# openai/Video-Pre-Training

Hardware: AMD Instinct MI355X
Metric: frames/sec (fwd) [+ bc_step.ms_per_step], 2x policy, 128x128x3 seq=128 (higher is better)
Workload: dtype bf16; 1 GPU; foundation-model-2x policy forward (IMPALA CNN + 4-layer banded transformer + heads), batch=64 seq=128 uint8 128x128x3 frames per GPU, KV memory carried, random-init weights; global_batch=64, seq_len=128, parallelism=dp1 replicas (no collective in forward; BC step: gradient all-reduce)

## Files before the change

### video-pre-training_amd/csrc/vpt_transformer.hip

```cpp
#include "vpt_common.h"
#include "vpt_kernels.h"

__global__ __launch_bounds__(256) void vpt_layernorm_kernel(VptLayerNormArgs a) {
  const int lane = threadIdx.x & 63;
  const int row = blockIdx.x * 4 + (threadIdx.x >> 6);
  if (row >= a.M) return;
  const float* x = a.x + (size_t)row * a.D;
  const int n4 = a.D >> 2;
  float s = 0.f;
  for (int i = lane; i < n4; i += 64) {
    f32x4 v = *(const f32x4*)(x + 4 * i);
    if (a.relu_in) { v.x = fmaxf(v.x, 0.f); v.y = fmaxf(v.y, 0.f); v.z = fmaxf(v.z, 0.f); v.w = fmaxf(v.w, 0.f); }
    s += (v.x + v.y) + (v.z + v.w);
  }
  const float mean = wave_sum(s) / (float)a.D;
  float ss = 0.f;
  for (int i = lane; i < n4; i += 64) {
    f32x4 v = *(const f32x4*)(x + 4 * i);
    if (a.relu_in) { v.x = fmaxf(v.x, 0.f); v.y = fmaxf(v.y, 0.f); v.z = fmaxf(v.z, 0.f); v.w = fmaxf(v.w, 0.f); }
    const float d0 = v.x - mean, d1 = v.y - mean, d2 = v.z - mean, d3 = v.w - mean;
    ss += (d0 * d0 + d1 * d1) + (d2 * d2 + d3 * d3);
  }
  const float rstd = rsqrtf(wave_sum(ss) / (float)a.D + VPT_NORM_EPS);
  for (int i = lane; i < n4; i += 64) {
    f32x4 v = *(const f32x4*)(x + 4 * i);
    if (a.relu_in) { v.x = fmaxf(v.x, 0.f); v.y = fmaxf(v.y, 0.f); v.z = fmaxf(v.z, 0.f); v.w = fmaxf(v.w, 0.f); }
    const f32x4 g = *(const f32x4*)(a.gain + 4 * i), b = *(const f32x4*)(a.bias + 4 * i);
    f32x4 y;
    y.x = fmaf((v.x - mean) * rstd, g.x, b.x);
    y.y = fmaf((v.y - mean) * rstd, g.y, b.y);
    y.z = fmaf((v.z - mean) * rstd, g.z, b.z);
    y.w = fmaf((v.w - mean) * rstd, g.w, b.w);
    if (a.out_f32) *(f32x4*)(a.out_f32 + (size_t)row * a.D + 4 * i) = y;
    if (a.out_bf16) {
      u32x2 p = {pack_op16x2(y.x, y.y), pack_op16x2(y.z, y.w)};
      *(u32x2*)(a.out_bf16 + (size_t)row * a.D + 4 * i) = p;
    }
  }
}

extern "C" int vpt_layernorm_launch(const VptLayerNormArgs* a, hipStream_t stream) {
  if (a->M <= 0 || (a->D & 3)) return -1;
  hipLaunchKernelGGL(vpt_layernorm_kernel, dim3((a->M + 3) >> 2), dim3(256), 0, stream, *a);
  return hipGetLastError() == hipSuccess ? 0 : -3;
}

#define ATT_DH 128
#define ATT_QT 32
#define ATT_NK 160
#define ATT_RS (ATT_DH + 4)
#define ATT_SS 164
#define ATT_S_OFF 0
#define ATT_R_OFF (ATT_S_OFF + ATT_QT * ATT_SS)
#define ATT_B_OFF (ATT_R_OFF + ATT_QT * 10)
#define ATT_SC_OFF (ATT_B_OFF + 10 * 129)
#define ATT_QL_OFF (ATT_SC_OFF + ATT_QT)
#define ATT_PT_OFF ((ATT_QL_OFF + ATT_QT + 3) & ~3)
#define ATT_FLOATS (ATT_PT_OFF + 4 * 16 * 64)

__global__ __launch_bounds__(256) void vpt_attn_kernel(VptAttnArgs a) {
  extern __shared__ __attribute__((aligned(16))) float sm[];
  float* Ss = sm + ATT_S_OFF;
  float* Rs = sm + ATT_R_OFF;
  float* Bs = sm + ATT_B_OFF;
  float* Sc = sm + ATT_SC_OFF;
  int* Ql = (int*)(sm + ATT_QL_OFF);

  const int tid = threadIdx.x, lane = tid & 63, w = __builtin_amdgcn_readfirstlane(tid >> 6);
  const int b = blockIdx.y / a.heads, h = blockIdx.y - b * a.heads;
  const int q0 = blockIdx.x * ATT_QT;
  const int maxlen = a.maxlen, t = a.t, hid = a.hid;
  const size_t tok0 = (size_t)b * t;
  const int jbase = a.causal ? q0 + 1 : 0;

  for (int idx = tid; idx < ATT_QT * 10; idx += 256) {
    const int r = idx / 10, n = idx - r * 10;
    Rs[idx] = (a.causal && q0 + r < t) ? a.qkvr[(tok0 + q0 + r) * a.ld + 3 * hid + h * 10 + n] : 0.f;
  }
  for (int idx = tid; idx < 10 * maxlen; idx += 256) Bs[idx] = a.b_nd[idx];
  if (tid < ATT_QT) Ql[tid] = (a.qlo && q0 + tid < t) ? a.qlo[tok0 + q0 + tid] : 0;
  __syncthreads();

  const int l31 = lane & 31, hi = lane >> 5;
  auto kv_row = [&](int j, int which) -> const float* {
    if (j < maxlen) return (which == 1 ? a.kmem : a.vmem) + ((size_t)b * maxlen + j) * hid + h * ATT_DH;
    if (j - maxlen < t) return a.qkvr + (tok0 + j - maxlen) * a.ld + which * hid + h * ATT_DH;
    return nullptr;
  };
  {
    f32x16 acc, acc4;
#pragma unroll
    for (int r = 0; r < 16; ++r) { acc[r] = 0.f; acc4[r] = 0.f; }
    const f32x4 z4 = {0.f, 0.f, 0.f, 0.f};
    const float* qa = (q0 + l31 < t) ? a.qkvr + (tok0 + q0 + l31) * a.ld + h * ATT_DH + 4 * hi : nullptr;
    const float* kr = kv_row(jbase + w * 32 + l31, 1);
    const float* kr4 = kv_row(jbase + 128 + l31, 1);
    const float* kb = kr ? kr + 4 * hi : nullptr;
    const float* kb4 = kr4 ? kr4 + 4 * hi : nullptr;
#pragma unroll 8
    for (int g = 0; g < 16; ++g) {
      const f32x4 q4 = qa ? *(const f32x4*)(qa + 8 * g) : z4, k4 = kb ? *(const f32x4*)(kb + 8 * g) : z4;
      acc = __builtin_amdgcn_mfma_f32_32x32x2f32(q4.x, k4.x, acc, 0, 0, 0);
      acc = __builtin_amdgcn_mfma_f32_32x32x2f32(q4.y, k4.y, acc, 0, 0, 0);
      acc = __builtin_amdgcn_mfma_f32_32x32x2f32(q4.z, k4.z, acc, 0, 0, 0);
      acc = __builtin_amdgcn_mfma_f32_32x32x2f32(q4.w, k4.w, acc, 0, 0, 0);
    }
#pragma unroll
    for (int g4 = 0; g4 < 4; ++g4) {
      const int g = 4 * w + g4;
      const f32x4 q4 = qa ? *(const f32x4*)(qa + 8 * g) : z4, k4 = kb4 ? *(const f32x4*)(kb4 + 8 * g) : z4;
      acc4 = __builtin_amdgcn_mfma_f32_32x32x2f32(q4.x, k4.x, acc4, 0, 0, 0);
      acc4 = __builtin_amdgcn_mfma_f32_32x32x2f32(q4.y, k4.y, acc4, 0, 0, 0);
      acc4 = __builtin_amdgcn_mfma_f32_32x32x2f32(q4.z, k4.z, acc4, 0, 0, 0);
      acc4 = __builtin_amdgcn_mfma_f32_32x32x2f32(q4.w, k4.w, acc4, 0, 0, 0);
    }
    float* Pt = sm + ATT_PT_OFF;
#pragma unroll
    for (int r = 0; r < 16; ++r) Pt[(w * 16 + r) * 64 + lane] = acc4[r];
    __syncthreads();
    auto finish = [&](int kk, int r, float dot) {
      const int qi = (r & 3) + 8 * (r >> 2) + 4 * hi;
      const bool qvalid = (q0 + qi) < t;
      const int off = maxlen - 1 + qi - kk;
      const int j = jbase + kk;
      bool vis = a.causal ? (qvalid && off >= 0 && off < maxlen) : (qvalid && kk < t);
      if (vis && a.causal && j < maxlen) vis = a.memvalid[(size_t)b * maxlen + j] != 0;
      vis = vis && j >= Ql[qi];
      float sc = -3.0e38f;
      if (vis) {
        float rb = 0.f;
        if (a.causal) {
#pragma unroll
          for (int n = 0; n < 10; ++n) rb = fmaf(Rs[qi * 10 + n], Bs[n * maxlen + off], rb);
        }
        sc = dot * (1.0f / ATT_DH) + rb;
      }
      Ss[qi * ATT_SS + kk] = sc;
    };
#pragma unroll
    for (int r = 0; r < 16; ++r) finish(w * 32 + l31, r, acc[r]);
#pragma unroll
    for (int r4 = 0; r4 < 4; ++r4) {
      const int r = 4 * w + r4;
      const float dot = (Pt[(0 * 16 + r) * 64 + lane] + Pt[(1 * 16 + r) * 64 + lane]) + (Pt[(2 * 16 + r) * 64 + lane] + Pt[(3 * 16 + r) * 64 + lane]);
      finish(128 + l31, r, dot);
    }
  }
  __syncthreads();
  for (int r = w * 8; r < w * 8 + 8; ++r) {
    float* srow = Ss + r * ATT_SS;
    const float s0 = srow[lane], s1 = srow[lane + 64], s2 = (lane + 128 < ATT_NK) ? srow[lane + 128] : -3.0e38f;
    const float m = wave_max(fmaxf(s0, fmaxf(s1, s2)));
    const float e0 = (s0 > -1.0e38f) ? expf(s0 - m) : 0.f;
    const float e1 = (s1 > -1.0e38f) ? expf(s1 - m) : 0.f;
    const float e2 = (s2 > -1.0e38f) ? expf(s2 - m) : 0.f;
    const float tot = wave_sum(e0 + e1 + e2);
    srow[lane] = e0;
    srow[lane + 64] = e1;
    if (lane + 128 < ATT_NK) srow[lane + 128] = e2;
    if (lane == 0) Sc[r] = (tot > 0.f) ? 1.0f / tot : 0.f;
  }
  __syncthreads();

  {
    f32x16 o;
#pragma unroll
    for (int r = 0; r < 16; ++r) o[r] = 0.f;
    const float* pa = Ss + l31 * ATT_SS + 4 * hi;
    const int dcol = w * 32 + l31;
#pragma unroll 4
    for (int g = 0; g < ATT_NK / 8; ++g) {
      const f32x4 p4 = *(const f32x4*)(pa + 8 * g);
      float v[4];
#pragma unroll
      for (int e = 0; e < 4; ++e) {
        const float* r0 = kv_row(jbase + 8 * g + e, 2);
        const float* r1 = kv_row(jbase + 8 * g + 4 + e, 2);
        const float* rr = hi ? r1 : r0;
        v[e] = rr ? rr[dcol] : 0.f;
      }
      o = __builtin_amdgcn_mfma_f32_32x32x2f32(p4.x, v[0], o, 0, 0, 0);
      o = __builtin_amdgcn_mfma_f32_32x32x2f32(p4.y, v[1], o, 0, 0, 0);
      o = __builtin_amdgcn_mfma_f32_32x32x2f32(p4.z, v[2], o, 0, 0, 0);
      o = __builtin_amdgcn_mfma_f32_32x32x2f32(p4.w, v[3], o, 0, 0, 0);
    }
#pragma unroll
    for (int r = 0; r < 16; ++r) {
      const int qi = (r & 3) + 8 * (r >> 2) + 4 * hi;
      if (q0 + qi < t) a.out[(tok0 + q0 + qi) * hid + h * ATT_DH + w * 32 + l31] = (vpt_op16)(o[r] * Sc[qi]);
    }
  }
}

extern "C" int vpt_attn_launch(const VptAttnArgs* a, hipStream_t stream) {
  if (a->hid != a->heads * ATT_DH) return -1;
  if (a->causal ? (a->maxlen < 1 || a->maxlen > 129) : (a->maxlen != 0 || a->t > ATT_NK)) return -1;
  if (a->qlo && !a->causal) return -1;
  static unsigned long long optin_done = 0;
  const size_t lds = ATT_FLOATS * sizeof(float);
  if (!vpt_lds_optin((const void*)vpt_attn_kernel, (int)lds, &optin_done)) return -4;
  dim3 grid((a->t + ATT_QT - 1) / ATT_QT, a->B * a->heads);
  hipLaunchKernelGGL(vpt_attn_kernel, grid, dim3(256), lds, stream, *a);
  return hipGetLastError() == hipSuccess ? 0 : -3;
}

struct VptAttnStepExtra {
  const uint8_t* state_mask;
  const uint8_t* first;
  uint8_t* mask_out;
  float* kout;
  float* vout;
  int* done;
};

__global__ __launch_bounds__(256) void vpt_attn_step_kernel(VptAttnArgs a, VptAttnStepExtra x) {
  __shared__ float sc_[128], red_[8], part_[128];
  __shared__ int last_;
  const int tid = threadIdx.x, lane = tid & 63, w = tid >> 6;
  const int b = blockIdx.x / a.heads, h = blockIdx.x - b * a.heads;
  const int maxlen = a.maxlen, hid = a.hid;
  const float* qrow = a.qkvr + (size_t)b * a.ld;
  auto kv_row = [&](int j, int which) -> const float* {
    if (j < maxlen) return (which == 1 ? a.kmem : a.vmem) + ((size_t)b * maxlen + j) * hid + h * ATT_DH;
    return qrow + which * hid + h * ATT_DH;
  };
  const int kk = tid >> 1, half = tid & 1;
  const bool live = kk < maxlen;
  const int j = 1 + kk;
  f32x4 kv[16];
  float s = -3.0e38f;
  bool vis = false;
  if (live) {
    const float* kr = kv_row(j, 1) + half * 64;
    const float* q = qrow + h * ATT_DH + half * 64;
    f32x4 qv[16];
#pragma unroll
    for (int i = 0; i < 16; ++i) kv[i] = *(const f32x4*)(kr + 4 * i);
#pragma unroll
    for (int i = 0; i < 16; ++i) qv[i] = *(const f32x4*)(q + 4 * i);
    const unsigned char mv = x.state_mask[(size_t)b * maxlen + min(j, maxlen - 1)];
    const unsigned char fst = x.first[b];
    const int off = maxlen - 1 - kk;
    float rr[10], bb[10];
#pragma unroll
    for (int n = 0; n < 10; ++n) { rr[n] = qrow[3 * hid + h * 10 + n]; bb[n] = a.b_nd[n * maxlen + off]; }
    float dot = 0.f;
#pragma unroll
    for (int i = 0; i < 16; ++i) {
      dot = fmaf(qv[i].x, kv[i].x, dot); dot = fmaf(qv[i].y, kv[i].y, dot); dot = fmaf(qv[i].z, kv[i].z, dot); dot = fmaf(qv[i].w, kv[i].w, dot);
    }
    dot += __shfl_xor(dot, 1, 64);
    vis = (j < maxlen) ? (mv != 0 && fst == 0) : true;
    if (vis) {
      float rb = 0.f;
#pragma unroll
      for (int n = 0; n < 10; ++n) rb = fmaf(rr[n], bb[n], rb);
      s = dot * (1.0f / ATT_DH) + rb;
    }
  }
  float m = wave_max(s);
  if (lane == 0) red_[w] = m;
  __syncthreads();
  if (live) {
    float* ko = x.kout + ((size_t)b * maxlen + kk) * hid + h * ATT_DH + half * 64;
#pragma unroll
    for (int i = 0; i < 16; ++i) *(f32x4*)(ko + 4 * i) = kv[i];
    if (!x.done && h == 0 && half == 0) x.mask_out[(size_t)b * maxlen + kk] = vis ? 1 : 0;
  }
  if (x.done && tid == 0) {
    __threadfence();
    const int arrived = atomicAdd(x.done + b, 1);
    last_ = (arrived == a.heads - 1);
    if (last_) x.done[b] = 0;
  }
  m = fmaxf(fmaxf(red_[0], red_[1]), fmaxf(red_[2], red_[3]));
  const float e = (s > -1.0e38f) ? expf(s - m) : 0.f;
  const float tot_w = wave_sum(half == 0 ? e : 0.f);
  if (half == 0) sc_[kk] = e;
  if (lane == 0) red_[4 + w] = tot_w;
  __syncthreads();
  const float tot = (red_[4] + red_[5]) + (red_[6] + red_[7]);
  const float inv = (tot > 0.f) ? 1.0f / tot : 0.f;
  if (x.done && last_ && live && half == 0) x.mask_out[(size_t)b * maxlen + kk] = vis ? 1 : 0;
  {
    const int d = tid & 127, kh = tid >> 7;
    const int k0 = kh * 64;
    float v[64];
#pragma unroll
    for (int i = 0; i < 64; ++i) v[i] = kv_row(1 + min(k0 + i, maxlen - 1), 2)[d];
    float o = 0.f;
    int cnt = __builtin_amdgcn_readfirstlane(maxlen - k0);
#pragma unroll
    for (int i = 0; i < 64; ++i)
      if (i < cnt) o = fmaf(sc_[k0 + i], v[i], o);
    if (kh == 1) part_[d] = o;
    __syncthreads();
    asm volatile("" : "+s"(cnt));
#pragma unroll
    for (int i = 0; i < 64; ++i)
      if (i < cnt) x.vout[((size_t)b * maxlen + k0 + i) * hid + h * ATT_DH + d] = v[i];
    if (kh == 0) a.out[(size_t)b * hid + h * ATT_DH + d] = (vpt_op16)((o + part_[d]) * inv);
  }
}

extern "C" int vpt_attn_step_launch(const VptAttnArgs* a, const uint8_t* state_mask, const uint8_t* first, uint8_t* mask_out, float* kout, float* vout,
                                    int* done, hipStream_t stream) {
  if (a->hid != a->heads * ATT_DH || a->t != 1 || !a->causal || a->maxlen < 1 || a->maxlen > 128) return -1;
  if (!kout || !vout || !state_mask || !first || !mask_out || (mask_out == state_mask && !done)) return -1;
  VptAttnStepExtra x;
  x.state_mask = state_mask; x.first = first; x.mask_out = mask_out; x.kout = kout; x.vout = vout; x.done = done;
  hipLaunchKernelGGL(vpt_attn_step_kernel, dim3((unsigned)(a->B * a->heads)), dim3(256), 0, stream, *a, x);
  return hipGetLastError() == hipSuccess ? 0 : -3;
}

__global__ __launch_bounds__(64) void vpt_episode_bounds_kernel(const uint8_t* first, const uint8_t* state_mask, int32_t* qlo, uint8_t* mask_out,
                                                                int t, int maxlen) {
  const int b = blockIdx.x, lane = threadIdx.x;
  const uint8_t* f = first + (size_t)b * t;
  int carry = -1;
  for (int p0 = 0; p0 < t; p0 += 64) {
    const int p = p0 + lane;
    const bool fl = p < t && f[p] != 0;
    const unsigned long long flags = __ballot(fl);
    const unsigned long long below = flags & (~0ull >> (63 - lane));
    const int s = below ? p0 + 63 - __clzll((long long)below) : carry;
    if (qlo && p < t) qlo[(size_t)b * t + p] = s >= 0 ? maxlen + s : 0;
    if (flags) carry = p0 + 63 - __clzll((long long)flags);
  }
  if (mask_out) {
    const int lo = carry >= 0 ? maxlen + carry : 0;
    for (int r = lane; r < maxlen; r += 64) {
      const long j = (long)t + r;
      mask_out[(size_t)b * maxlen + r] = (j >= lo && (j >= maxlen || state_mask[(size_t)b * maxlen + j] != 0)) ? 1 : 0;
    }
  }
}

extern "C" int vpt_episode_bounds_launch(const uint8_t* first, const uint8_t* state_mask, int32_t* qlo, uint8_t* mask_out, int B, int t, int maxlen,
                                         hipStream_t stream) {
  if (!first || B <= 0 || t < 1 || maxlen < 1 || (long)t + maxlen > 0x7fffffffL) return -1;
  if (mask_out && (!state_mask || mask_out == state_mask)) return -1;
  if (!qlo && !mask_out) return 0;
  hipLaunchKernelGGL(vpt_episode_bounds_kernel, dim3((unsigned)B), dim3(64), 0, stream, first, state_mask, qlo, mask_out, t, maxlen);
  return hipGetLastError() == hipSuccess ? 0 : -3;
}

__global__ __launch_bounds__(256) void vpt_kv_update_kernel(VptKvUpdateArgs a) {
  const int which = blockIdx.y;
  const size_t n4 = (size_t)a.B * a.maxlen * (a.hid >> 2);
  const size_t idx = (size_t)blockIdx.x * 256 + threadIdx.x;
  if (idx >= n4) return;
  const int h4 = a.hid >> 2;
  const int c4 = (int)(idx % h4);
  const size_t rs = idx / h4;
  const int s = (int)(rs % a.maxlen);
  const int b = (int)(rs / a.maxlen);
  const int src = s + a.t;
  const float* mem = which ? a.vmem : a.kmem;
  float* out = which ? a.vout : a.kout;
  f32x4 v;
  if (src < a.maxlen) v = *(const f32x4*)(mem + ((size_t)b * a.maxlen + src) * a.hid + c4 * 4);
  else v = *(const f32x4*)(a.qkvr + ((size_t)b * a.t + (src - a.maxlen)) * a.ld + (which ? 2 : 1) * a.hid + c4 * 4);
  *(f32x4*)(out + ((size_t)b * a.maxlen + s) * a.hid + c4 * 4) = v;
}

extern "C" int vpt_kv_update_launch(const VptKvUpdateArgs* a, hipStream_t stream) {
  if (a->B <= 0 || (a->hid & 3)) return -1;
  const size_t n4 = (size_t)a->B * a->maxlen * (a->hid >> 2);
  dim3 grid((unsigned)((n4 + 255) / 256), 2);
  hipLaunchKernelGGL(vpt_kv_update_kernel, grid, dim3(256), 0, stream, *a);
  return hipGetLastError() == hipSuccess ? 0 : -3;
}

#define LSM_CAP 9
template <int NW>
__global__ __launch_bounds__(64 * NW) void vpt_logsoftmax_kernel(VptLogSoftmaxArgs a) {
  constexpr int NT = 64 * NW;
  __shared__ float red[3 * NW];
  __shared__ int redi[NW];
  const int row = blockIdx.x, tid = threadIdx.x, lane = tid & 63, w = tid >> 6;
  const float* z = a.logits + (size_t)row * a.ld + a.col0;
  const uint8_t* mk = a.mask ? a.mask + (size_t)row * a.n : nullptr;
  const float T = a.temperature;
#define SCALED(i_) ((mk && !mk[i_]) ? -100.0f : z[i_] / T)
  float c[LSM_CAP];
  float m = -3.0e38f;
#pragma unroll
  for (int k = 0; k < LSM_CAP; ++k) {
    const int i = tid + NT * k;
    c[k] = (i < a.n) ? SCALED(i) : -3.0e38f;
    m = fmaxf(m, c[k]);
  }
  for (int i = tid + NT * LSM_CAP; i < a.n; i += NT) m = fmaxf(m, SCALED(i));
  m = wave_max(m);
  if (lane == 0) red[w] = m;
  __syncthreads();
  m = red[0];
#pragma unroll
  for (int k = 1; k < NW; ++k) m = fmaxf(m, red[k]);
  float s = 0.f;
#pragma unroll
  for (int k = 0; k < LSM_CAP; ++k) s += (tid + NT * k < a.n) ? expf(c[k] - m) : 0.f;
  for (int i = tid + NT * LSM_CAP; i < a.n; i += NT) s += expf(SCALED(i) - m);
  s = wave_sum(s);
  if (lane == 0) red[NW + w] = s;
  __syncthreads();
  float tot = 0.f;
#pragma unroll
  for (int k = 0; k < NW; ++k) tot += red[NW + k];
  const float lse = m + logf(tot);
  float* o = a.out + (size_t)row * a.n;
  const float* u = a.noise ? a.noise + (size_t)row * a.n : nullptr;
  const bool gen = !u && a.rng_state != nullptr;
  uint64_t seed = 0, rstep = 0;
  if (gen) { seed = a.rng_state[0]; rstep = a.rng_state[1]; }
  float best = -3.0e38f;
  int besti = 0x7fffffff;
  auto emit = [&](int i, float sc_) __attribute__((always_inline)) {
    const float lp = sc_ - lse;
    o[i] = lp;
    if (a.action) {
      float sc = lp;
      if (u || gen) {
        float ui = u ? u[i] : vpt_philox_uniform(seed, rstep, a.rng_stream, (uint32_t)row, (uint32_t)i);
        if (ui == 1.0f) ui = 0.999f;
        sc = lp - logf(-logf(ui));
      }
      if (sc > best) { best = sc; besti = i; }
    }
  };
#pragma unroll
  for (int k = 0; k < LSM_CAP; ++k)
    if (tid + NT * k < a.n) emit(tid + NT * k, c[k]);
  for (int i = tid + NT * LSM_CAP; i < a.n; i += NT) emit(i, SCALED(i));
  if (a.action) {
#pragma unroll
    for (int off = 32; off > 0; off >>= 1) {
      const float ob = __shfl_xor(best, off, 64);
      const int oi = __shfl_xor(besti, off, 64);
      if (ob > best || (ob == best && oi < besti)) { best = ob; besti = oi; }
    }
    if (lane == 0) { red[2 * NW + w] = best; redi[w] = besti; }
    __syncthreads();
    if (tid == 0) {
      for (int k = 1; k < NW; ++k)
        if (red[2 * NW + k] > best || (red[2 * NW + k] == best && redi[k] < besti)) { best = red[2 * NW + k]; besti = redi[k]; }
      if (besti >= a.n) besti = 0;
      a.action[row] = besti;
      if (a.action_logp) a.action_logp[row] = ((mk && !mk[besti]) ? -100.0f : z[besti] / T) - lse;
    }
  }
#undef SCALED
}

extern "C" int vpt_logsoftmax_launch(const VptLogSoftmaxArgs* a, hipStream_t stream) {
  if (a->M <= 0 || a->n <= 0) return -1;
  if (a->M < 64 && a->n > 1024) hipLaunchKernelGGL((vpt_logsoftmax_kernel<16>), dim3(a->M), dim3(1024), 0, stream, *a);
  else hipLaunchKernelGGL((vpt_logsoftmax_kernel<4>), dim3(a->M), dim3(256), 0, stream, *a);
  return hipGetLastError() == hipSuccess ? 0 : -3;
}

__global__ void vpt_act_epilogue_kernel(const int64_t* act_b, const int64_t* act_c, const float* lp_b, const float* lp_c, const float* logits, int ld,
                                        int vcol, float scale, float shift, int64_t* keep, uint8_t* nan_flag, uint64_t* rng_state, int B) {
  const int b = threadIdx.x;
  bool bad = false;
  if (b < B) {
    const float lp = lp_b[b] + lp_c[b];
    const float v = logits[(size_t)b * ld + vcol];
    const float vd = fmaf(v, scale, shift);
    bad = lp != lp;
    keep[4 * b + 0] = act_b[b];
    keep[4 * b + 1] = act_c[b];
    keep[4 * b + 2] = (int64_t)(uint64_t)__builtin_bit_cast(uint32_t, lp);
    keep[4 * b + 3] = (int64_t)((uint64_t)__builtin_bit_cast(uint32_t, vd) | ((uint64_t)__builtin_bit_cast(uint32_t, v) << 32));
  }
  const unsigned long long any = __ballot(bad);
  if (threadIdx.x == 0) {
    *nan_flag = any ? 1 : 0;
    if (rng_state) rng_state[1] += 1;
  }
}

__global__ __launch_bounds__(256) void vpt_uniform_noise_kernel(const uint64_t* rng_state, uint32_t rng_stream, float* out, int M, int n) {
  const uint64_t seed = rng_state[0], rstep = rng_state[1];
  const long total = (long)M * n;
  for (long idx = (long)blockIdx.x * 256 + threadIdx.x; idx < total; idx += (long)gridDim.x * 256) {
    const int row = (int)(idx / n), i = (int)(idx - (long)row * n);
    out[idx] = vpt_philox_uniform(seed, rstep, rng_stream, (uint32_t)row, (uint32_t)i);
  }
}

extern "C" int vpt_uniform_noise_launch(const uint64_t* rng_state, uint32_t rng_stream, float* out, int M, int n, hipStream_t stream) {
  if (!rng_state || !out || M <= 0 || n <= 0) return -1;
  const long total = (long)M * n;
  const unsigned grid = (unsigned)((total + 255) / 256 > 4096 ? 4096 : (total + 255) / 256);
  hipLaunchKernelGGL(vpt_uniform_noise_kernel, dim3(grid), dim3(256), 0, stream, rng_state, rng_stream, out, M, n);
  return hipGetLastError() == hipSuccess ? 0 : -3;
}

extern "C" int vpt_act_epilogue_launch(const int64_t* act_b, const int64_t* act_c, const float* lp_b, const float* lp_c, const float* logits, int ld,
                                       int vcol, float scale, float shift, int64_t* keep, uint8_t* nan_flag, uint64_t* rng_state, int B, hipStream_t stream) {
  if (B <= 0 || B > 64 || !keep || !nan_flag) return -1;
  hipLaunchKernelGGL(vpt_act_epilogue_kernel, dim3(1), dim3(64), 0, stream, act_b, act_c, lp_b, lp_c, logits, ld, vcol, scale, shift, keep, nan_flag, rng_state, B);
  return hipGetLastError() == hipSuccess ? 0 : -3;
}
```

Measured before the change: 81080 frames/s.

## Prefetch Q/K/V into registers and LDS up front in attention kernel; batch softmax reductions

The attention kernel now issues all global loads for Q, K, V, the relative-bias terms and the memory-valid mask before the first barrier. Q is staged in LDS and K/V are held in registers, so load latency overlaps the setup and the QK and PV MFMA loops no longer wait on global reads. The visibility logic is made branchless and specialized on the causal flag. Softmax row reductions are interleaved four rows at a time, the launch bounds request 3 blocks per CU, and the logsoftmax cache capacity grows for the 4-wave variant. These changes raise register pressure substantially, which may cause spills or lower occupancy.

```diff
diff --git a/video-pre-training_amd/csrc/vpt_transformer.hip b/video-pre-training_amd/csrc/vpt_transformer.hip
--- a/video-pre-training_amd/csrc/vpt_transformer.hip
+++ b/video-pre-training_amd/csrc/vpt_transformer.hip
@@ -58,7 +58,7 @@
 #define ATT_PT_OFF ((ATT_QL_OFF + ATT_QT + 3) & ~3)
 #define ATT_FLOATS (ATT_PT_OFF + 4 * 16 * 64)
 
-__global__ __launch_bounds__(256) void vpt_attn_kernel(VptAttnArgs a) {
+__global__ __launch_bounds__(256, 3) void vpt_attn_kernel(VptAttnArgs a) {
   extern __shared__ __attribute__((aligned(16))) float sm[];
   float* Ss = sm + ATT_S_OFF;
   float* Rs = sm + ATT_R_OFF;
@@ -73,33 +73,61 @@
   const size_t tok0 = (size_t)b * t;
   const int jbase = a.causal ? q0 + 1 : 0;
 
-  for (int idx = tid; idx < ATT_QT * 10; idx += 256) {
-    const int r = idx / 10, n = idx - r * 10;
-    Rs[idx] = (a.causal && q0 + r < t) ? a.qkvr[(tok0 + q0 + r) * a.ld + 3 * hid + h * 10 + n] : 0.f;
-  }
-  for (int idx = tid; idx < 10 * maxlen; idx += 256) Bs[idx] = a.b_nd[idx];
-  if (tid < ATT_QT) Ql[tid] = (a.qlo && q0 + tid < t) ? a.qlo[tok0 + q0 + tid] : 0;
-  __syncthreads();
-
   const int l31 = lane & 31, hi = lane >> 5;
   auto kv_row = [&](int j, int which) -> const float* {
     if (j < maxlen) return (which == 1 ? a.kmem : a.vmem) + ((size_t)b * maxlen + j) * hid + h * ATT_DH;
     if (j - maxlen < t) return a.qkvr + (tok0 + j - maxlen) * a.ld + which * hid + h * ATT_DH;
     return nullptr;
   };
+  const f32x4 z4 = {0.f, 0.f, 0.f, 0.f};
+  float* Qs = sm + ATT_S_OFF;
+  f32x4 qst[4];
+  float rst[2], bst[6];
+#pragma unroll
+  for (int i = 0; i < 4; ++i) {
+    const int r = (tid >> 5) + 8 * i;
+    qst[i] = (q0 + r < t) ? *(const f32x4*)(a.qkvr + (tok0 + q0 + r) * a.ld + h * ATT_DH + 4 * (tid & 31)) : z4;
+  }
+#pragma unroll
+  for (int i = 0; i < 2; ++i) {
+    const int idx = tid + 256 * i, r = idx / 10, n = idx - r * 10;
+    rst[i] = (idx < ATT_QT * 10 && a.causal && q0 + r < t) ? a.qkvr[(tok0 + q0 + r) * a.ld + 3 * hid + h * 10 + n] : 0.f;
+  }
+#pragma unroll
+  for (int i = 0; i < 6; ++i) bst[i] = (tid + 256 * i < 10 * maxlen) ? a.b_nd[tid + 256 * i] : 0.f;
+  const int qlst = (tid < ATT_QT && a.qlo && q0 + tid < t) ? a.qlo[tok0 + q0 + tid] : 0;
+  const int jlast = maxlen + t - 1, jk = jbase + w * 32 + l31, jk4 = jbase + 128 + l31;
+  const uint8_t* mvp = a.causal ? a.memvalid + (size_t)b * maxlen + min(jk, maxlen - 1) : (const uint8_t*)a.qkvr;
+  const uint8_t mvb = *mvp;
+  f32x4 kf[16], kf4[4];
+  {
+    const float* kr = kv_row(min(jk, jlast), 1) + 4 * hi;
+    const float* kr4 = kv_row(min(jk4, jlast), 1) + 4 * hi + 32 * w;
+#pragma unroll
+    for (int g = 0; g < 16; ++g) kf[g] = *(const f32x4*)(kr + 8 * g);
+#pragma unroll
+    for (int g4 = 0; g4 < 4; ++g4) kf4[g4] = *(const f32x4*)(kr4 + 8 * g4);
+  }
+#pragma unroll
+  for (int i = 0; i < 4; ++i) *(f32x4*)(Qs + ((tid >> 5) + 8 * i) * ATT_RS + 4 * (tid & 31)) = qst[i];
+#pragma unroll
+  for (int i = 0; i < 2; ++i)
+    if (tid + 256 * i < ATT_QT * 10) Rs[tid + 256 * i] = rst[i];
+#pragma unroll
+  for (int i = 0; i < 6; ++i)
+    if (tid + 256 * i < 10 * maxlen) Bs[tid + 256 * i] = bst[i];
+  if (tid < ATT_QT) Ql[tid] = qlst;
+  __syncthreads();
+
+  float vv[ATT_NK / 8][4];
   {
     f32x16 acc, acc4;
 #pragma unroll
     for (int r = 0; r < 16; ++r) { acc[r] = 0.f; acc4[r] = 0.f; }
-    const f32x4 z4 = {0.f, 0.f, 0.f, 0.f};
-    const float* qa = (q0 + l31 < t) ? a.qkvr + (tok0 + q0 + l31) * a.ld + h * ATT_DH + 4 * hi : nullptr;
-    const float* kr = kv_row(jbase + w * 32 + l31, 1);
-    const float* kr4 = kv_row(jbase + 128 + l31, 1);
-    const float* kb = kr ? kr + 4 * hi : nullptr;
-    const float* kb4 = kr4 ? kr4 + 4 * hi : nullptr;
-#pragma unroll 8
+    const float* qa = Qs + l31 * ATT_RS + 4 * hi;
+#pragma unroll
     for (int g = 0; g < 16; ++g) {
-      const f32x4 q4 = qa ? *(const f32x4*)(qa + 8 * g) : z4, k4 = kb ? *(const f32x4*)(kb + 8 * g) : z4;
+      const f32x4 q4 = *(const f32x4*)(qa + 8 * g), k4 = jk <= jlast ? kf[g] : z4;
       acc = __builtin_amdgcn_mfma_f32_32x32x2f32(q4.x, k4.x, acc, 0, 0, 0);
       acc = __builtin_amdgcn_mfma_f32_32x32x2f32(q4.y, k4.y, acc, 0, 0, 0);
       acc = __builtin_amdgcn_mfma_f32_32x32x2f32(q4.z, k4.z, acc, 0, 0, 0);
@@ -107,58 +135,99 @@
     }
 #pragma unroll
     for (int g4 = 0; g4 < 4; ++g4) {
-      const int g = 4 * w + g4;
-      const f32x4 q4 = qa ? *(const f32x4*)(qa + 8 * g) : z4, k4 = kb4 ? *(const f32x4*)(kb4 + 8 * g) : z4;
+      const f32x4 q4 = *(const f32x4*)(qa + 8 * (4 * w + g4)), k4 = jk4 <= jlast ? kf4[g4] : z4;
       acc4 = __builtin_amdgcn_mfma_f32_32x32x2f32(q4.x, k4.x, acc4, 0, 0, 0);
       acc4 = __builtin_amdgcn_mfma_f32_32x32x2f32(q4.y, k4.y, acc4, 0, 0, 0);
       acc4 = __builtin_amdgcn_mfma_f32_32x32x2f32(q4.z, k4.z, acc4, 0, 0, 0);
       acc4 = __builtin_amdgcn_mfma_f32_32x32x2f32(q4.w, k4.w, acc4, 0, 0, 0);
     }
+    {
+      typedef const __attribute__((address_space(1))) float* global_f32;
+      const int dcol = h * ATT_DH + w * 32 + l31;
+      const unsigned j0 = jbase + 4 * hi;
+      const uint64_t mem_bytes = 4u * hid, chunk_bytes = 4u * a.ld;
+      uint64_t pm = (uint64_t)a.vmem + 4 * ((uint64_t)b * maxlen * hid + dcol) + j0 * mem_bytes;
+      uint64_t pc = (uint64_t)a.qkvr + 4 * ((uint64_t)((int64_t)tok0 + j0 - maxlen) * a.ld + 2 * hid + dcol);
+#pragma unroll
+      for (int g = 0; g < ATT_NK / 8; ++g) {
+#pragma unroll
+        for (int e = 0; e < 4; ++e) {
+          const unsigned j = j0 + 8 * g + e;
+          vv[g][e] = (j < (unsigned)(maxlen + t)) ? *(global_f32)(j < (unsigned)maxlen ? pm : pc) : 0.f;
+          pm += (e < 3 ? 1 : 5) * mem_bytes;
+          pc += (e < 3 ? 1 : 5) * chunk_bytes;
+        }
+      }
+    }
     float* Pt = sm + ATT_PT_OFF;
 #pragma unroll
     for (int r = 0; r < 16; ++r) Pt[(w * 16 + r) * 64 + lane] = acc4[r];
     __syncthreads();
-    auto finish = [&](int kk, int r, float dot) {
+    auto finish = [&](const bool causal, int kk, int r, float dot, bool memvis) {
       const int qi = (r & 3) + 8 * (r >> 2) + 4 * hi;
       const bool qvalid = (q0 + qi) < t;
       const int off = maxlen - 1 + qi - kk;
       const int j = jbase + kk;
-      bool vis = a.causal ? (qvalid && off >= 0 && off < maxlen) : (qvalid && kk < t);
-      if (vis && a.causal && j < maxlen) vis = a.memvalid[(size_t)b * maxlen + j] != 0;
-      vis = vis && j >= Ql[qi];
-      float sc = -3.0e38f;
-      if (vis) {
-        float rb = 0.f;
-        if (a.causal) {
-#pragma unroll
-          for (int n = 0; n < 10; ++n) rb = fmaf(Rs[qi * 10 + n], Bs[n * maxlen + off], rb);
-        }
-        sc = dot * (1.0f / ATT_DH) + rb;
+      const int ql = Ql[qi];
+      const bool vis = (causal ? (qvalid & (off >= 0) & (off < maxlen)) : (qvalid & (kk < t))) & memvis & (j >= ql);
+      float rb = 0.f;
+      if (causal) {
+        const int offc = min(max(off, 0), maxlen - 1);
+#pragma unroll
+        for (int n = 0; n < 10; ++n) rb = fmaf(Rs[qi * 10 + n], Bs[n * maxlen + offc], rb);
       }
-      Ss[qi * ATT_SS + kk] = sc;
+      const float sc = dot * (1.0f / ATT_DH) + rb;
+      Ss[qi * ATT_SS + kk] = vis ? sc : -3.0e38f;
     };
-#pragma unroll
-    for (int r = 0; r < 16; ++r) finish(w * 32 + l31, r, acc[r]);
-#pragma unroll
-    for (int r4 = 0; r4 < 4; ++r4) {
-      const int r = 4 * w + r4;
-      const float dot = (Pt[(0 * 16 + r) * 64 + lane] + Pt[(1 * 16 + r) * 64 + lane]) + (Pt[(2 * 16 + r) * 64 + lane] + Pt[(3 * 16 + r) * 64 + lane]);
-      finish(128 + l31, r, dot);
-    }
-  }
-  __syncthreads();
-  for (int r = w * 8; r < w * 8 + 8; ++r) {
-    float* srow = Ss + r * ATT_SS;
-    const float s0 = srow[lane], s1 = srow[lane + 64], s2 = (lane + 128 < ATT_NK) ? srow[lane + 128] : -3.0e38f;
-    const float m = wave_max(fmaxf(s0, fmaxf(s1, s2)));
-    const float e0 = (s0 > -1.0e38f) ? expf(s0 - m) : 0.f;
-    const float e1 = (s1 > -1.0e38f) ? expf(s1 - m) : 0.f;
-    const float e2 = (s2 > -1.0e38f) ? expf(s2 - m) : 0.f;
-    const float tot = wave_sum(e0 + e1 + e2);
-    srow[lane] = e0;
-    srow[lane + 64] = e1;
-    if (lane + 128 < ATT_NK) srow[lane + 128] = e2;
-    if (lane == 0) Sc[r] = (tot > 0.f) ? 1.0f / tot : 0.f;
+    auto finish_all = [&](const bool causal) {
+      const bool memvis = !(causal && jk < maxlen) || mvb != 0;
+#pragma unroll
+      for (int r = 0; r < 16; ++r) finish(causal, w * 32 + l31, r, acc[r], memvis);
+#pragma unroll
+      for (int r4 = 0; r4 < 4; ++r4) {
+        const int r = 4 * w + r4;
+        const float dot = (Pt[(0 * 16 + r) * 64 + lane] + Pt[(1 * 16 + r) * 64 + lane]) + (Pt[(2 * 16 + r) * 64 + lane] + Pt[(3 * 16 + r) * 64 + lane]);
+        finish(causal, 128 + l31, r, dot, true);
+      }
+    };
+    if (a.causal) finish_all(true);
+    else finish_all(false);
+  }
+  __syncthreads();
+#pragma unroll
+  for (int r0 = w * 8; r0 < w * 8 + 8; r0 += 4) {
+    float s[4][3], e[4][3], m[4], tot[4];
+#pragma unroll
+    for (int i = 0; i < 4; ++i) {
+      const float* srow = Ss + (r0 + i) * ATT_SS;
+      s[i][0] = srow[lane];
+      s[i][1] = srow[lane + 64];
+      s[i][2] = (lane + 128 < ATT_NK) ? srow[lane + 128] : -3.0e38f;
+    }
+#pragma unroll
+    for (int i = 0; i < 4; ++i) m[i] = fmaxf(s[i][0], fmaxf(s[i][1], s[i][2]));
+#pragma unroll
+    for (int o = 32; o > 0; o >>= 1)
+#pragma unroll
+      for (int i = 0; i < 4; ++i) m[i] = fmaxf(m[i], __shfl_xor(m[i], o, 64));
+#pragma unroll
+    for (int i = 0; i < 4; ++i) {
+#pragma unroll
+      for (int c = 0; c < 3; ++c) e[i][c] = (s[i][c] > -1.0e38f) ? expf(s[i][c] - m[i]) : 0.f;
+      tot[i] = e[i][0] + e[i][1] + e[i][2];
+    }
+#pragma unroll
+    for (int o = 32; o > 0; o >>= 1)
+#pragma unroll
+      for (int i = 0; i < 4; ++i) tot[i] += __shfl_xor(tot[i], o, 64);
+#pragma unroll
+    for (int i = 0; i < 4; ++i) {
+      float* srow = Ss + (r0 + i) * ATT_SS;
+      srow[lane] = e[i][0];
+      srow[lane + 64] = e[i][1];
+      if (lane + 128 < ATT_NK) srow[lane + 128] = e[i][2];
+      if (lane == 0) Sc[r0 + i] = (tot[i] > 0.f) ? 1.0f / tot[i] : 0.f;
+    }
   }
   __syncthreads();
 
@@ -167,22 +236,13 @@
 #pragma unroll
     for (int r = 0; r < 16; ++r) o[r] = 0.f;
     const float* pa = Ss + l31 * ATT_SS + 4 * hi;
-    const int dcol = w * 32 + l31;
-#pragma unroll 4
+#pragma unroll
     for (int g = 0; g < ATT_NK / 8; ++g) {
       const f32x4 p4 = *(const f32x4*)(pa + 8 * g);
-      float v[4];
-#pragma unroll
-      for (int e = 0; e < 4; ++e) {
-        const float* r0 = kv_row(jbase + 8 * g + e, 2);
-        const float* r1 = kv_row(jbase + 8 * g + 4 + e, 2);
-        const float* rr = hi ? r1 : r0;
-        v[e] = rr ? rr[dcol] : 0.f;
-      }
-      o = __builtin_amdgcn_mfma_f32_32x32x2f32(p4.x, v[0], o, 0, 0, 0);
-      o = __builtin_amdgcn_mfma_f32_32x32x2f32(p4.y, v[1], o, 0, 0, 0);
-      o = __builtin_amdgcn_mfma_f32_32x32x2f32(p4.z, v[2], o, 0, 0, 0);
-      o = __builtin_amdgcn_mfma_f32_32x32x2f32(p4.w, v[3], o, 0, 0, 0);
+      o = __builtin_amdgcn_mfma_f32_32x32x2f32(p4.x, vv[g][0], o, 0, 0, 0);
+      o = __builtin_amdgcn_mfma_f32_32x32x2f32(p4.y, vv[g][1], o, 0, 0, 0);
+      o = __builtin_amdgcn_mfma_f32_32x32x2f32(p4.z, vv[g][2], o, 0, 0, 0);
+      o = __builtin_amdgcn_mfma_f32_32x32x2f32(p4.w, vv[g][3], o, 0, 0, 0);
     }
 #pragma unroll
     for (int r = 0; r < 16; ++r) {
@@ -372,10 +432,10 @@
   return hipGetLastError() == hipSuccess ? 0 : -3;
 }
 
-#define LSM_CAP 9
+#define LSM_CAP(NW_) ((NW_) == 4 ? 34 : 9)
 template <int NW>
 __global__ __launch_bounds__(64 * NW) void vpt_logsoftmax_kernel(VptLogSoftmaxArgs a) {
-  constexpr int NT = 64 * NW;
+  constexpr int NT = 64 * NW, CAP = LSM_CAP(NW);
   __shared__ float red[3 * NW];
   __shared__ int redi[NW];
   const int row = blockIdx.x, tid = threadIdx.x, lane = tid & 63, w = tid >> 6;
@@ -383,25 +443,27 @@
   const uint8_t* mk = a.mask ? a.mask + (size_t)row * a.n : nullptr;
   const float T = a.temperature;
 #define SCALED(i_) ((mk && !mk[i_]) ? -100.0f : z[i_] / T)
-  float c[LSM_CAP];
+  float c[CAP];
   float m = -3.0e38f;
 #pragma unroll
-  for (int k = 0; k < LSM_CAP; ++k) {
+  for (int k = 0; k < CAP; ++k) {
     const int i = tid + NT * k;
     c[k] = (i < a.n) ? SCALED(i) : -3.0e38f;
     m = fmaxf(m, c[k]);
   }
-  for (int i = tid + NT * LSM_CAP; i < a.n; i += NT) m = fmaxf(m, SCALED(i));
+  for (int i = tid + NT * CAP; i < a.n; i += NT) m = fmaxf(m, SCALED(i));
   m = wave_max(m);
   if (lane == 0) red[w] = m;
   __syncthreads();
   m = red[0];
 #pragma unroll
   for (int k = 1; k < NW; ++k) m = fmaxf(m, red[k]);
+  int n2 = a.n;
+  asm volatile("" : "+s"(n2));
   float s = 0.f;
 #pragma unroll
-  for (int k = 0; k < LSM_CAP; ++k) s += (tid + NT * k < a.n) ? expf(c[k] - m) : 0.f;
-  for (int i = tid + NT * LSM_CAP; i < a.n; i += NT) s += expf(SCALED(i) - m);
+  for (int k = 0; k < CAP; ++k) s += (tid + NT * k < n2) ? expf(c[k] - m) : 0.f;
+  for (int i = tid + NT * CAP; i < a.n; i += NT) s += expf(SCALED(i) - m);
   s = wave_sum(s);
   if (lane == 0) red[NW + w] = s;
   __syncthreads();
@@ -429,10 +491,12 @@
       if (sc > best) { best = sc; besti = i; }
     }
   };
-#pragma unroll
-  for (int k = 0; k < LSM_CAP; ++k)
-    if (tid + NT * k < a.n) emit(tid + NT * k, c[k]);
-  for (int i = tid + NT * LSM_CAP; i < a.n; i += NT) emit(i, SCALED(i));
+  int n3 = a.n;
+  asm volatile("" : "+s"(n3));
+#pragma unroll
+  for (int k = 0; k < CAP; ++k)
+    if (tid + NT * k < n3) emit(tid + NT * k, c[k]);
+  for (int i = tid + NT * CAP; i < a.n; i += NT) emit(i, SCALED(i));
   if (a.action) {
 #pragma unroll
     for (int off = 32; off > 0; off >>= 1) {
```

Result: no change. 81660 frames/s (median of 6 runs) (+0.7%).
